# dkogan/libdogleg

Hardware: AMD Instinct MI355X
Metric: trust-region steps/sec (fp64) at fixed (Nmeas,Nstate,nnz) (higher is better)
Workload: dtype f64

## Files before the change

### libdogleg_amd/csrc/sparse_factor.hip

```cpp
#include "sparse_internal.h"
#include "panel_factor.h"
#include "factor_tail.h"

namespace {
#ifdef DLG_FL_PROFILE
constexpr int FL_PROF_WG = 4096;
__device__ long long g_fl_prof[32*FL_PROF_WG*8];
__device__ long long g_fl_add[FL_PROF_WG*4];
#define FL_ADD_STAMP(k) do { if(HANDOFF && threadIdx.x == 0 && blockIdx.x < FL_PROF_WG) g_fl_add[blockIdx.x*4 + (k)] = wall_clock64(); } while(0)
#define FL_STAMP(k) do { if(threadIdx.x == 0 && blockIdx.x < FL_PROF_WG) g_fl_prof[((prof_lvl & 31)*FL_PROF_WG + blockIdx.x)*8 + (k)] = wall_clock64(); } while(0)
#else
#define FL_STAMP(k)
#define FL_ADD_STAMP(k)
#endif

template <int NT, bool UT_LDS, bool HANDOFF = false>
__device__ __forceinline__ void mf_add_children(double* P, double* Wt, int ntri, int nch, int ch0,
                                                MfChild rc, const MfChild* __restrict__ mf_rec,
                                                const double* uscr, const uint16_t* __restrict__ mf_dst, int tid,
                                                int* pr_flag = nullptr, int pr_epoch = 0, DlgHandoff ho = DlgHandoff{nullptr, 0, 0}, int z0 = 0)
{
  constexpr int MF_SLOTS = (NT >= 512) ? 20 : 16;
  const int lane = tid & 63;
  for(int e = z0 + tid; e < ntri; e += NT) Wt[e] = 0.0;
// ... 513 lines not shown
  const double* Ld = Lx + sn_lx[d] + wd;
  double* U = uscr + u_off[d];
  const int T = (mb + 15) >> 4, MB16 = T*16;
  const int LDB = ((mb + 31)/32)*32 + 16, K4 = (wd + 3) & ~3;
  const int tid = threadIdx.x, lane = tid & 63;
  const int w = __builtin_amdgcn_readfirstlane(tid >> 6);
  const int jn = lane & 15, kq = lane >> 4;
  const int ntiles = T*(T + 1)/2;
  int aoff[TPW], boff[TPW];
#pragma unroll
  for(int q = 0; q < TPW; q++)
  {
    int rem = w + q*NW, tj = 0;
    if(rem < ntiles) { while(rem >= T - tj) { rem -= T - tj; tj++; } }
    else { rem = 0; tj = 0; }
    aoff[q] = 16*(tj + rem); boff[q] = 16*tj;
  }
  const int nmine = (ntiles - w + NW - 1)/NW;
  dlg_v4d c4[TPW];
#pragma unroll
  for(int q = 0; q < TPW; q++) c4[q] = (dlg_v4d){0.0, 0.0, 0.0, 0.0};
  for(int k0 = 0; k0 < K4; k0 += KC)
  {
    const int kc = min(KC, K4 - k0);
    if(k0 > 0) __syncthreads();
    batched_copy<NT, 8>(kc*MB16, tid,
                        [&](int e) { const int k = k0 + e / MB16, i = e % MB16; return (k < wd && i < mb) ? Ld[i + (size_t)k*nrows] : 0.0; },
                        [&](int e, double v) { const int k = e / MB16, i = e - k*MB16; Bs[k*LDB + i] = v; });
    __syncthreads();
    const double* base = Bs + kq*LDB + jn;
#pragma unroll 2
    for(int kk = 0; kk < kc; kk += 4)
    {
#pragma unroll
      for(int q = 0; q < TPW; q++)
        if(q < nmine)
          c4[q] = __builtin_amdgcn_mfma_f64_16x16x4f64(base[kk*LDB + aoff[q]], base[kk*LDB + boff[q]], c4[q], 0, 0, 0);
    }
  }
#pragma unroll
  for(int q = 0; q < TPW; q++)
    if(q < nmine)
    {
      const int j = boff[q] + jn;
#pragma unroll
      for(int r = 0; r < 4; r++)
      {
        const int i = aoff[q] + kq + 4*r;
        if(i < mb && j <= i) U[tri_col(j, mb) + i] = c4[q][r];
      }
    }
}
constexpr int GATHER_FLIGHT = 4;
template <int NT>
__global__ void __launch_bounds__(NT) k_update_gather(int unit0, const GatherUnit* __restrict__ units,
                                                       const SymSub* __restrict__ usub,
                                                       const int64_t* __restrict__ usub_u,
                                                       const int* __restrict__ relpos,
                                                       double* __restrict__ Lx,
                                                       double* __restrict__ upart,
                                                       const double* __restrict__ uscr, int nw,
                                                       int* __restrict__ info,
                                                       const int* __restrict__ fin_gate = nullptr, int fin_epoch = 0, int* fin_status = nullptr)
{
  extern __shared__ __attribute__((aligned(16))) double lds[];
  __shared__ int s_skip;
  int fin_seen = fin_epoch;
  if(fin_gate && threadIdx.x == 0) fin_seen = __hip_atomic_load(fin_gate, __ATOMIC_RELAXED, __HIP_MEMORY_SCOPE_AGENT);
  if(threadIdx.x == 0)
  {
    s_skip = *info != 0x7fffffff;
  }
  const GatherUnit U0 = units[unit0 + blockIdx.x];
  const int nc = U0.nc, nrows_t = U0.nrows_t, s0 = U0.s0, s1 = U0.s1;
  double* Lt = Lx + U0.lt;
  const int64_t part = U0.part;
  const int tid = threadIdx.x, lane = tid & 63;
  const int w = __builtin_amdgcn_readfirstlane(tid >> 6);
  const int slab = nrows_t*nc;
  for(int e = tid; e < slab*nw; e += NT) lds[e] = 0.0;
  __syncthreads();
  if(s_skip) return;
  if(w < nw)
  {
    double* acc = lds + (size_t)w*slab;
    const int nmine = (s1 - s0 - w + nw - 1)/nw;
    for(int k0 = 0; k0 < nmine; k0 += 64)
    {
      const int stl = s0 + w + (k0 + min(lane, nmine - k0 - 1))*nw;
      const SymSub R = usub[stl];
      const int64_t ru = usub_u[stl];
      const int r_rel = R.rel, r_mb = R.nrows_d - R.wd, r_m = R.m;
      const int r_ulo = (int)(uint32_t)ru, r_uhi = (int)(ru >> 32);
      const int nb = min(64, nmine - k0);
      for(int k = 0; k < nb; k += GATHER_FLIGHT)
      {
        int relv[GATHER_FLIGHT], mbv[GATHER_FLIGHT], mv[GATHER_FLIGHT], mmax = 0;
        const double* Uv[GATHER_FLIGHT];
#pragma unroll
        for(int g = 0; g < GATHER_FLIGHT; g++)
        {
          const int kg = min(k + g, nb - 1);
          relv[g] = __builtin_amdgcn_readlane(r_rel, kg);
          mbv[g] = __builtin_amdgcn_readlane(r_mb, kg);
          mv[g] = (k + g < nb) ? __builtin_amdgcn_readlane(r_m, kg) : 0;
          Uv[g] = uscr + (int64_t)(((uint64_t)(uint32_t)__builtin_amdgcn_readlane(r_uhi, kg) << 32) | (uint32_t)__builtin_amdgcn_readlane(r_ulo, kg));
          mmax = max(mmax, mv[g]);
        }
        int mv2[GATHER_FLIGHT];
#pragma unroll
        for(int g = 0; g < GATHER_FLIGHT; g++) mv2[g] = max(mv[g], 1);
        for(int i0 = 0; i0 < mmax; i0 += 64)
        {
          const int i = i0 + lane;
          const int cmax = (i < nc - 1) ? i : nc - 1;
          int ig[GATHER_FLIGHT], rg[GATHER_FLIGHT];
          double v[GATHER_FLIGHT][8];
#pragma unroll
          for(int g = 0; g < GATHER_FLIGHT; g++) { ig[g] = min(i, max(mv[g], 1) - 1); rg[g] = relpos[relv[g] + ig[g]]; }
#pragma unroll
          for(int g = 0; g < GATHER_FLIGHT; g++)
#pragma unroll
            for(int c = 0; c < 8; c++)
              if(c < nc) { const int cc = min(min(c, cmax), ig[g]); v[g][c] = Uv[g][ig[g] + cc*(mv2[g] - 1) - cc*(cc - 1)/2]; }
#pragma unroll
          for(int g = 0; g < GATHER_FLIGHT; g++)
#pragma unroll
            for(int c = 0; c < 8; c++)
              if(c < nc) { if(i < mv[g] && c <= cmax) acc[rg[g] + c*nrows_t] += v[g][c]; }
        }
      }
    }
  }
  if(fin_gate && tid == 0)
    for(int spins = 0; fin_seen != fin_epoch; spins++)
    {
      if(spins > (1 << 21)) { atomicOr(fin_status, DLG_HANDOFF_FACTOR); break; }
      __builtin_amdgcn_s_sleep(8);
      fin_seen = __hip_atomic_load(fin_gate, __ATOMIC_ACQUIRE, __HIP_MEMORY_SCOPE_AGENT);
    }
  __syncthreads();
  for(int e0 = tid; e0 < slab; e0 += 8*NT)
  {
    double old[8], tot[8];
#pragma unroll
    for(int u = 0; u < 8; u++) old[u] = (part < 0 && e0 + u*NT < slab) ? Lt[e0 + u*NT] : 0.0;
#pragma unroll
    for(int u = 0; u < 8; u++)
    {
      tot[u] = 0.0;
      if(e0 + u*NT < slab) for(int k = 0; k < nw; k++) tot[u] += lds[(size_t)k*slab + e0 + u*NT];
    }
#pragma unroll
    for(int u = 0; u < 8; u++)
      if(e0 + u*NT < slab) { if(part < 0) Lt[e0 + u*NT] = old[u] - tot[u]; else upart[part + e0 + u*NT] = tot[u]; }
  }
}

constexpr int UPD_TILES = 6;
__global__ void __launch_bounds__(TPB) k_update_mfma(int unit0, const int* __restrict__ uw_item,
                                                     const int* __restrict__ uw_s0,
                                                     const int* __restrict__ uw_s1,
                                                     const int64_t* __restrict__ uw_part,
                                                     const int* __restrict__ ui_t,
                                                     const int* __restrict__ ui_col,
                                                     const int* __restrict__ ui_nc,
                                                     const SymSub* __restrict__ usub,
                                                     const int* __restrict__ relpos,
                                                     const int* __restrict__ sn_rowptr,
                                                     const int64_t* __restrict__ sn_lx,
                                                     double* __restrict__ Lx,
                                                     double* __restrict__ upart, int nw, const int* __restrict__ info)
{
  extern __shared__ __attribute__((aligned(16))) double lds[];
  if(*info != 0x7fffffff) return;

  const int unit = unit0 + blockIdx.x;
  const int item = uw_item[unit];
  const int t = ui_t[item], col = ui_col[item], nc = ui_nc[item];
  const int nrows_t = sn_rowptr[t+1] - sn_rowptr[t];
  double* Lt = Lx + sn_lx[t] + (int64_t)col*nrows_t;
  const int s0 = uw_s0[unit], s1 = uw_s1[unit];
  const int64_t part = uw_part[unit];
  const int tid = threadIdx.x, lane = tid & 63;
  const int w = __builtin_amdgcn_readfirstlane(tid >> 6);
  const int slab = nrows_t*nc;
  for(int e = tid; e < slab*nw; e += TPB) lds[e] = 0.0;
  __syncthreads();
  if(w < nw)
  {
    double* acc = lds + (size_t)w*slab;
    const int jn = lane & 15, kq = lane >> 4;
    const int jc = min(jn, nc - 1);
    int piece = 0;
    for(int st = s0; st < s1; st++)
    {
      const SymSub U = usub[st];
      const double* Ld = Lx + U.src;
      const int* rel = relpos + U.rel;
      const int ld = U.nrows_d, wd = U.wd, m = U.m;
      for(int mt0 = 0; mt0 < m; mt0 += 16*UPD_TILES, piece++)
      {
        if(piece % nw != w) continue;
        const int ntile = min(UPD_TILES, (m - mt0 + 15) >> 4);
        const int relv0 = rel[min(mt0 + lane, m - 1)], relv1 = rel[min(mt0 + 64 + lane, m - 1)];
        dlg_v4d c4[UPD_TILES];
#pragma unroll
        for(int q = 0; q < UPD_TILES; q++) c4[q] = (dlg_v4d){0.0, 0.0, 0.0, 0.0};
        int ia[UPD_TILES];
// ... 100 lines not shown
            const double ai = Ld[i + (size_t)q*ld];
#pragma unroll
            for(int c = 0; c < 8; c++) if(c <= cmax) sacc[c] += ai*Ld[c + (size_t)q*ld];
          }
          const int r = rel[i];
#pragma unroll
          for(int c = 0; c < 8; c++) if(c <= cmax) acc[r + c*nrows_t] += sacc[c];
        }
      }
    }
    __syncthreads();
    for(int e = tid; e < slab; e += TPB)
    {
      double tot = 0.0;
      for(int k = 0; k < nw; k++) tot += lds[(size_t)k*slab + e];
      if(part < 0) Lt[e] -= tot; else upart[part + e] = tot;
    }
  }
  else
  {
    double* dst = (part < 0) ? Lt : upart + part;
    const double sgn = (part < 0) ? -1.0 : 1.0;
    if(part >= 0) { for(int e = tid; e < slab; e += TPB) dst[e] = 0.0; __syncthreads(); }
    for(int st = s0; st < s1; st++)
    {
      const SymSub U = usub[st];
      const double* Ld = Lx + U.src;
      const int* rel = relpos + U.rel;
      const int ld = U.nrows_d;
      for(int i = tid; i < U.m; i += TPB)
      {
        const int cmax = (i < nc - 1) ? i : nc - 1;
        const int r = rel[i];
        for(int c = 0; c <= cmax; c++)
        {
          double sacc = 0.0;
          for(int q = 0; q < U.wd; q++) sacc += Ld[i + (size_t)q*ld]*Ld[c + (size_t)q*ld];
          dst[r + c*nrows_t] += sgn*sacc;
        }
      }
      __syncthreads();
    }
  }
}
__global__ void __launch_bounds__(TPB) k_update_fin(int f0, const int* __restrict__ uf_item,
                                                    const int* __restrict__ uf_n,
                                                    const int64_t* __restrict__ uf_off,
                                                    const int* __restrict__ ui_t,
                                                    const int* __restrict__ ui_col,
                                                    const int* __restrict__ ui_nc,
                                                    const int* __restrict__ sn_rowptr,
                                                    const int64_t* __restrict__ sn_lx,
                                                    double* __restrict__ Lx,
                                                    const double* __restrict__ upart, const int* __restrict__ info)
{
  __shared__ double sh[TPB];
  if(*info != 0x7fffffff) return;

  const int f = f0 + blockIdx.x;
  const int item = uf_item[f], n = uf_n[f];
  const int t = ui_t[item], col = ui_col[item], nc = ui_nc[item];
  const int nrows_t = sn_rowptr[t+1] - sn_rowptr[t];
  double* Lt = Lx + sn_lx[t] + (int64_t)col*nrows_t;
  const int slab = nrows_t*nc;
  const double* src = upart + uf_off[f];
  const int E = (slab >= 32) ? 32 : 8;
  const int G = TPB/E;
  const int el = threadIdx.x % E, g = threadIdx.x / E;
  for(int ebase = blockIdx.y*E; ebase < slab; ebase += gridDim.y*E)
  {
    const int e = ebase + el;
    double t0 = 0.0, t1 = 0.0, t2 = 0.0, t3 = 0.0;
    if(e < slab)
    {
      const double* q = src + e;
      int k = g;
      for(; k + 3*G < n; k += 4*G)
      {
        t0 += q[(size_t)k*slab];         t1 += q[(size_t)(k + G)*slab];
        t2 += q[(size_t)(k + 2*G)*slab]; t3 += q[(size_t)(k + 3*G)*slab];
      }
      for(; k < n; k += G) t0 += q[(size_t)k*slab];
    }
    __syncthreads();
    sh[threadIdx.x] = (t0 + t1) + (t2 + t3);
    __syncthreads();
    if(g == 0 && e < slab)
    {
      double sacc = 0.0;
      for(int k = 0; k < G; k++) sacc += sh[k*E + el];
      Lt[e] -= sacc;
    }
  }
}

}

static int env_int_host(const char* n, int d) { const char* v = getenv(n); return v ? atoi(v) : d; }
int sparse_factor_setup(dlg_backend* b, bool plan_only)
{
  SparseSym* Y = b->sym;
  const SymHost& H = Y->H;
  Y->fac_b16 = true;
  Y->fac_lds.assign(H.nlevels, 0); Y->fac_nt.assign(H.nlevels, 512); Y->upd_coop.assign(H.nlevels, 0);
  Y->upd_lds.assign(H.nlevels, 0); Y->upd_nw.assign(H.nlevels, 0);
  Y->syrk_lds.assign(H.nlevels, 0); Y->syrk_nt.assign(H.nlevels, 256); Y->syrk_kc.assign(H.nlevels, 4);
  Y->syrk_fused.assign(H.nlevels, 0); Y->fin_ny.assign(H.nlevels, 1); Y->fac_stage.assign(H.nlevels, 0);
  Y->fac_leaf.assign(H.nlevels, 0);
  for(int l = 0; l < H.nlevels && !getenv("DOGLEG_AMD_NO_LEAF_KERNEL"); l++)
  {
    bool all = H.fw_lvl_ptr[l+1] > H.fw_lvl_ptr[l] && l < H.mf_level0;
    long maxr = 0;
// ... 53 lines not shown
    if(H.upd_syrk[l])
    {
      long ldbmax = 0, k4max = 0, tmax = 0;
      for(int i = H.lvl_ptr[l]; i < H.lvl_ptr[l+1]; i++)
      {
        const int d = H.lvl_sn[i];
        const long wd = H.sn_c0[d+1] - H.sn_c0[d], mb = H.sn_rowptr[d+1] - H.sn_rowptr[d] - wd;
        ldbmax = std::max(ldbmax, ((mb + 31)/32)*32 + 16); k4max = std::max(k4max, (wd + 3)/4*4);
        tmax = std::max(tmax, (mb + 15)/16);
      }
      long kc = (65536/(ldbmax*8)) & ~3L;
      if(kc > k4max) kc = k4max;
      Y->syrk_kc[l] = (int)kc;
      Y->syrk_lds[l] = (int)(kc*ldbmax*8);
      Y->syrk_nt[l] = (tmax*(tmax + 1)/2 <= 32) ? 256 : 1024;
      bool unsliced = true;
      for(int i = H.lvl_ptr[l]; i < H.lvl_ptr[l+1]; i++) if(H.sn_top[H.lvl_sn[i]] >= 0) unsliced = false;
      Y->syrk_fused[l] = (unsliced && nw > 0 && !getenv("DOGLEG_AMD_NO_SYRK_FUSE")) ? 1 : 0;
    }
    if(l >= H.mf_level0 || Y->syrk_fused[l])
    {
      long with_children = Y->fac_lds[l], leaves = Y->fac_lds[l];
      for(int i = H.lvl_ptr[l]; i < H.lvl_ptr[l+1]; i++)
      {
        const int s = H.lvl_sn[i];
        const long wv = H.sn_c0[s+1] - H.sn_c0[s], nr = H.sn_rowptr[s+1] - H.sn_rowptr[s], mb = nr - wv;
        const bool cmp = H.sn_bd_ptr[s+1] > H.sn_bd_ptr[s] && H.sn_top[s] < 0;
        const long pan = cmp ? ((mb + 1) & ~1L)*wv + (Y->fac_leaf[l] ? 4 : 8)*wv : ((nr + 1) & ~1L)*wv;
        const int jsp = cmp ? (int)mb : sym_w_split(wv, nr);
        const long need = (pan + (jsp >= 0 ? sym_w_linear(mb, jsp) : mb*(mb + 1)/2) + 1)*8;
        const long need0 = (pan + 1)*8;
        const long want = (need <= FAC_LDS_BUDGET && jsp >= 0) ? need : need0;
        const bool has_children = l >= H.mf_level0 && H.mf_cptr[s+1] > H.mf_cptr[s];
        if(has_children) with_children = std::max(with_children, want); else leaves = std::max(leaves, want);
      }
      const long base = std::max((long)Y->fac_lds[l], with_children);
      const long per_cu0 = 163840/(base + 3584), per_cu1 = 163840/(std::max(base, leaves) + 3584);
      Y->fac_stage[l] = (per_cu1 == per_cu0) ? 1 : 0;
      Y->fac_lds[l] = (int)(Y->fac_stage[l] ? std::max(base, leaves) : base);
    }
    if(getenv("DOGLEG_AMD_SYM_DEBUG"))
      fprintf(stderr, "factor level %d: %d supernodes, dynamic LDS %d bytes, update matrices staged %d, leaf instantiation %d, gather: %d waves, %d bytes\n",
              l, H.lvl_ptr[l+1] - H.lvl_ptr[l], Y->fac_lds[l], (int)Y->fac_stage[l], (int)Y->fac_leaf[l], Y->upd_nw[l], Y->upd_lds[l]);
  }
  if(!Y->uw_flat && !H.uw_item.empty() && !plan_only)
  {
    std::vector<GatherUnit> fl(H.uw_item.size());
    for(size_t u = 0; u < fl.size(); u++)
    {
      const int item = H.uw_item[u], t = H.ui_t[item];
      const int nr = H.sn_rowptr[t+1] - H.sn_rowptr[t];
      fl[u].lt = H.sn_lx[t] + (int64_t)H.ui_col[item]*nr; fl[u].part = H.uw_part[u];
      fl[u].s0 = H.uw_s0[u]; fl[u].s1 = H.uw_s1[u]; fl[u].nrows_t = nr; fl[u].nc = H.ui_nc[item];
    }
    DLG_CHECK(upload(Y->uw_flat, fl)); Y->allocs.push_back(Y->uw_flat);
  }
  Y->pr_level0 = H.nlevels; Y->pr2_level0 = H.nlevels; Y->pr2_level1 = -1;
  const bool dbg = getenv("DOGLEG_AMD_TIMING") != nullptr;
  bool acc_any = false;
  auto build_region = [&](int lo_min, int hi, int& r_level0, int& r_lds, int& r_stage, int& r_nwg,
                          std::vector<FwItem>& items, std::vector<MfChild>& rec, std::vector<uint16_t>& dst) -> int
  {
    r_level0 = H.nlevels; r_nwg = 0;
    if(getenv("DOGLEG_AMD_NO_PERSIST") || H.nlevels < 2 || hi < lo_min) return DLG_OK;
    const int ncu = b->ncu;
    const int cap = env_int_host("DOGLEG_AMD_PERSIST_MAX", 5*ncu);
    int total = 0, l0 = hi + 1, lds = 0, stage = 1;
    const int nt = Y->fac_nt[hi];
    for(int l = hi; l >= std::max(1, lo_min); l--)
    {
      const int n = H.fw_lvl_ptr[l+1] - H.fw_lvl_ptr[l];
      if(l < H.mf_level0) break;
      if(n == 0 || total + n > cap || Y->fac_nt[l] != nt || Y->fac_lds[l] <= 0) break;
      if(H.uw_lvl_ptr[l+1] > H.uw_lvl_ptr[l] || H.uf_lvl_ptr[l+1] > H.uf_lvl_ptr[l]) break;
      bool ok = true;
      for(int i = H.fw_lvl_ptr[l]; i < H.fw_lvl_ptr[l+1] && ok; i++)
      {
        const FwItem& it = H.fw_item[i];
        if(it.top >= 0 || it.r0 != 0 || it.nbd > 0) ok = false;
      }
      if(!ok) break;
      stage = stage && Y->fac_stage[l]; total += n; l0 = l; lds = std::max(lds, Y->fac_lds[l]);
    }
    if(hi + 1 - l0 < 2) return DLG_OK;
    r_level0 = l0; r_lds = lds; r_stage = stage;
    {
      const int rmax = std::max(1, std::min(8, env_int_host("DOGLEG_AMD_FRONT_REPLICAS", 8)));
      const int fill = ncu/2, fill0 = ncu/2;
      const bool slice_ok = !getenv("DOGLEG_AMD_NO_FRONT_SLICES");
      std::vector<int> first(H.fw_item.size(), -1), count(H.fw_item.size(), 0);
      rec = H.mf_rec; dst = H.mf_dst;
      auto lin = [](long j, long mb) { return j*mb - j*(j - 1)/2; };
      long lds_need = lds;
      std::vector<double> est(H.fw_item.size(), 0.0);
      std::vector<int> item_of_sn(H.nsn, -1);
      for(int l = r_level0; l <= hi; l++)
        for(int i = H.fw_lvl_ptr[l]; i < H.fw_lvl_ptr[l+1]; i++) item_of_sn[H.fw_sn[i]] = i;
      for(int l = r_level0; l <= hi; l++)
      {
        const int n = H.fw_lvl_ptr[l+1] - H.fw_lvl_ptr[l];
        std::vector<int> order(n);
        for(int k = 0; k < n; k++) order[k] = H.fw_lvl_ptr[l] + k;
        for(int i : order)
        {
          const FwItem& fi = H.fw_item[i];
          double e0 = 0.0;
// ... 171 lines not shown
      std::vector<FwItem> items2; std::vector<MfChild> rec2; std::vector<uint16_t> dst2;
      DLG_CHECK(build_region(1, H.cut_level, Y->pr2_level0, Y->pr2_lds, Y->pr2_stage, Y->pr2_nwg, items2, rec2, dst2));
      if(Y->pr2_level0 <= H.cut_level)
      {
        Y->pr2_level1 = H.cut_level;
        if(!Y->pr2_item) { DLG_CHECK(upload(Y->pr2_item, items2)); Y->allocs.push_back(Y->pr2_item); }
        if(!Y->pr2_rec)  { DLG_CHECK(upload(Y->pr2_rec, rec2));   Y->allocs.push_back(Y->pr2_rec); }
        if(!Y->pr2_dst)  { DLG_CHECK(upload(Y->pr2_dst, dst2));   Y->allocs.push_back(Y->pr2_dst); }
      }
      else Y->pr2_level0 = H.nlevels;
    }
    if(acc_any && !Y->pr_acc && !plan_only)
    {
      DLG_HIP(hipMalloc(&Y->pr_acc, sizeof(double)*(size_t)std::max<int64_t>(1, H.uscr_size)));
      Y->allocs.push_back(Y->pr_acc);
    }
  }
  if(plan_only) return DLG_OK;
  if(Y->pr_level0 < H.nlevels && !Y->fac_flag)
  {
    DLG_HIP(hipMalloc(&Y->fac_flag, sizeof(int)*((size_t)Y->pr_nwg + 1)));
    Y->allocs.push_back(Y->fac_flag);
    DLG_HIP(hipMemsetAsync(Y->fac_flag, 0, sizeof(int)*((size_t)Y->pr_nwg + 1), b->stream));
    Y->fac_epoch = 0;
  }
  if(Y->pr2_level0 < H.nlevels && !Y->fac2_flag)
  {
    DLG_HIP(hipMalloc(&Y->fac2_flag, sizeof(int)*((size_t)Y->pr2_nwg + 1)));
    Y->allocs.push_back(Y->fac2_flag);
    DLG_HIP(hipMemsetAsync(Y->fac2_flag, 0, sizeof(int)*((size_t)Y->pr2_nwg + 1), b->stream));
    Y->fac2_epoch = 0;
  }
  DLG_HIP(hipFuncSetAttribute(reinterpret_cast<const void*>(&k_factor_level<128>),
                              hipFuncAttributeMaxDynamicSharedMemorySize, FAC_LDS_BUDGET));
  DLG_HIP(hipFuncSetAttribute(reinterpret_cast<const void*>(&k_factor_level<256>),
                              hipFuncAttributeMaxDynamicSharedMemorySize, FAC_LDS_BUDGET));
  DLG_HIP(hipFuncSetAttribute(reinterpret_cast<const void*>(&k_factor_level<256, true>),
                              hipFuncAttributeMaxDynamicSharedMemorySize, FAC_LDS_BUDGET));
  DLG_HIP(hipFuncSetAttribute(reinterpret_cast<const void*>(&k_factor_level<512>),
                              hipFuncAttributeMaxDynamicSharedMemorySize, FAC_LDS_BUDGET));
  DLG_HIP(hipFuncSetAttribute(reinterpret_cast<const void*>(&k_update_level),
                              hipFuncAttributeMaxDynamicSharedMemorySize, LDS_BUDGET));
  DLG_HIP(hipFuncSetAttribute(reinterpret_cast<const void*>(&k_update_syrk<256>),
                              hipFuncAttributeMaxDynamicSharedMemorySize, LDS_BUDGET));
  DLG_HIP(hipFuncSetAttribute(reinterpret_cast<const void*>(&k_update_syrk<1024>),
                              hipFuncAttributeMaxDynamicSharedMemorySize, LDS_BUDGET));
  DLG_HIP(hipFuncSetAttribute(reinterpret_cast<const void*>(&k_update_gather<TPB>),
                              hipFuncAttributeMaxDynamicSharedMemorySize, LDS_BUDGET));
  DLG_HIP(hipFuncSetAttribute(reinterpret_cast<const void*>(&k_update_mfma),
                              hipFuncAttributeMaxDynamicSharedMemorySize, LDS_BUDGET));
  return DLG_OK;
}

#ifdef DLG_FL_PROFILE
extern "C" void dlg_fl_profile_dump(int nlevels)
{
  std::vector<long long> h(32*FL_PROF_WG*8);
  hipDeviceSynchronize();
  hipMemcpyFromSymbol(h.data(), HIP_SYMBOL(g_fl_prof), sizeof(long long)*h.size());
  for(int l = 0; l < nlevels && l < 32; l++)
  {
    int nwg = 0, last = -1; long long t0 = 0, tend = 0; double mean[5] = {0, 0, 0, 0, 0};
    for(int g = 0; g < FL_PROF_WG; g++)
    {
      const long long* q = &h[(l*FL_PROF_WG + g)*8];
      if(q[5] == 0) continue;
      nwg++;
      if(t0 == 0 || q[0] < t0) t0 = q[0];
      if(q[5] > tend) { tend = q[5]; last = g; }
      for(int k = 0; k < 5; k++) mean[k] += (double)(q[k+1] - q[k]);
    }
    if(nwg == 0) continue;
    for(int g = FL_PROF_WG - 1, shown = 0; g >= 0 && shown < (getenv("DLG_FL_DUMP_ALL") ? FL_PROF_WG : 20); g--)
    {
      const long long* q = &h[(l*FL_PROF_WG + g)*8];
      if(q[5] == 0 || q[7] == 0) continue;
      shown++;
      {
        std::vector<long long> ha(FL_PROF_WG*4);
        static bool got = false; static std::vector<long long> hadd;
        if(!got) { hadd.resize(FL_PROF_WG*4); hipMemcpyFromSymbol(hadd.data(), HIP_SYMBOL(g_fl_add), sizeof(long long)*hadd.size()); got = true; }
        if(hadd[g*4 + 0]) fprintf(stderr, "   add %3d: child0 seen %6lld child0 added %6lld last child seen %6lld dbg %lld\n", g, hadd[g*4] - t0, hadd[g*4 + 1] - t0, hadd[g*4 + 2] - t0, hadd[g*4 + 3]);
      }
      fprintf(stderr, "   wg %3d (w %3lld rows %4lld nch %lld u_lds %lld lvl %lld rep %lld): start %6lld flag up %6lld panel in %6lld added %6lld factored %6lld tail %6lld flag+stored %6lld\n",
              g, q[6] & 4095, (q[6] >> 12) & 4095, (q[6] >> 24) & 4095, (q[6] >> 36) & 1, (q[6] >> 56) & 63, (q[6] >> 52) & 15, q[0] - t0, q[7] - t0, q[1] - t0, q[2] - t0, q[3] - t0, q[4] - t0, q[5] - t0);
    }
    const long long* q = &h[(l*FL_PROF_WG + last)*8];
    fprintf(stderr, "level %2d: %3d wg, span %7lld | last wg %3d (w %3lld rows %4lld slice %4lld nch %2lld u_lds %lld has_u %lld): start +%6lld load %6lld add %6lld factor %6lld tail %6lld store %6lld | mean: load %6.0f add %6.0f factor %6.0f tail %6.0f store %6.0f\n",
            l, nwg, tend - t0, last, q[6] & 4095, (q[6] >> 12) & 4095, (q[6] >> 40) & 4095, (q[6] >> 24) & 4095, (q[6] >> 36) & 1, (q[6] >> 37) & 1,
            q[0] - t0, q[1] - q[0], q[2] - q[1], q[3] - q[2], q[4] - q[3], q[5] - q[4],
            mean[0]/nwg, mean[1]/nwg, mean[2]/nwg, mean[3]/nwg, mean[4]/nwg);
  }
  std::vector<long long> z(h.size(), 0);
  hipMemcpyToSymbol(HIP_SYMBOL(g_fl_prof), z.data(), sizeof(long long)*z.size());
}
#endif
int sparse_factor_levels(dlg_backend* b, int part)
{
  SparseSym* Y = b->sym;
  const SymHost& H = Y->H;
  hipStream_t st = b->stream;
  const bool split = Y->pr_level0 > 0 && H.nlevels >= 2 && H.part_nranks <= 1 && H.fw_lvl_ptr[1] > H.fw_lvl_ptr[0];
  if(part == 2 && !split) return DLG_OK;
  if(part != 2)
  {
  if(H.part_nranks > 1 && H.cut_level < 0) DLG_CHECK(sparse_partition_reduce(b));
// ... 40 lines not shown
      const DlgHandoff ho = dlg_handoff(b, 1 << 21);
      DlgRegionTurn turn(b);
      if(Y->fac_nt[l] == 128)
        hipLaunchKernelGGL(HIP_KERNEL_NAME(k_factor_level<128>), dim3(np), dim3(128), Y->pr_lds, st,
                           Y->pr_item, Y->pr_rec, Y->sn_bd_col, Y->pr_dst, Y->Lx, Y->top_scr, Y->d_info, Y->uscr, fmode, fl, ep, ho, pacc);
      else if(Y->fac_nt[l] == 256)
        hipLaunchKernelGGL(HIP_KERNEL_NAME(k_factor_level<256>), dim3(np), dim3(256), Y->pr_lds, st,
                           Y->pr_item, Y->pr_rec, Y->sn_bd_col, Y->pr_dst, Y->Lx, Y->top_scr, Y->d_info, Y->uscr, fmode, fl, ep, ho, pacc);
      else
        hipLaunchKernelGGL(HIP_KERNEL_NAME(k_factor_level<512>), dim3(np), dim3(512), Y->pr_lds, st,
                           Y->pr_item, Y->pr_rec, Y->sn_bd_col, Y->pr_dst, Y->Lx, Y->top_scr, Y->d_info, Y->uscr, fmode, fl, ep, ho, pacc);
      break;
    }
    if(n > 0 && !launched_before)
    {
      const int o = H.fw_lvl_ptr[l];
      const int sweep_bits = (Y->fac_b16 ? 16 : 0);
      const int fmode = ((l >= H.mf_level0) ? 2 : Y->syrk_fused[l]) + 4*Y->fac_stage[l] + sweep_bits + 256*(l & 31);
      if(Y->fac_nt[l] == 128)
        hipLaunchKernelGGL(HIP_KERNEL_NAME(k_factor_level<128>), dim3(n), dim3(128), Y->fac_lds[l], st,
                           Y->fw_item + o, Y->mf_rec, Y->sn_bd_col, Y->mf_dst, Y->Lx, Y->top_scr, Y->d_info, Y->uscr, fmode, (int*)nullptr, 0, DlgHandoff{nullptr, 0, 0}, (int64_t)0);
      else if(Y->fac_nt[l] == 256 && Y->fac_leaf[l])
        hipLaunchKernelGGL(HIP_KERNEL_NAME(k_factor_level<256, true>), dim3(n), dim3(256), Y->fac_lds[l], st,
                           Y->fw_item + o, Y->mf_rec, Y->sn_bd_col, Y->mf_dst, Y->Lx, Y->top_scr, Y->d_info, Y->uscr, fmode, (int*)nullptr, 0, DlgHandoff{nullptr, 0, 0}, (int64_t)0);
      else if(Y->fac_nt[l] == 256)
        hipLaunchKernelGGL(HIP_KERNEL_NAME(k_factor_level<256>), dim3(n), dim3(256), Y->fac_lds[l], st,
                           Y->fw_item + o, Y->mf_rec, Y->sn_bd_col, Y->mf_dst, Y->Lx, Y->top_scr, Y->d_info, Y->uscr, fmode, (int*)nullptr, 0, DlgHandoff{nullptr, 0, 0}, (int64_t)0);
      else
        hipLaunchKernelGGL(HIP_KERNEL_NAME(k_factor_level<512>), dim3(n), dim3(512), Y->fac_lds[l], st,
                           Y->fw_item + o, Y->mf_rec, Y->sn_bd_col, Y->mf_dst, Y->Lx, Y->top_scr, Y->d_info, Y->uscr, fmode, (int*)nullptr, 0, DlgHandoff{nullptr, 0, 0}, (int64_t)0);
    }
    if(part == 1 && split && l == 0) { Y->fac_pending = true; DLG_LAUNCH_CHECK(); return DLG_OK; }
    const int nu = H.uw_lvl_ptr[l+1] - H.uw_lvl_ptr[l];
    const bool gather_next = nu > 0 && H.upd_syrk[l] && Y->upd_nw[l] > 0;
    const int fin_ep = (l == 0 && gather_next) ? Y->fin_side_owed : 0;
    if(fin_ep) Y->fin_side_owed = 0;
    if(l == 0) DLG_CHECK(sparse_fin_side_gate(b));
    if(gather_next)
    {
      const int ns = H.xl_ptr[l+1] - H.xl_ptr[l];
      if(Y->syrk_fused[l] || ns == 0) {  }
      else if(Y->syrk_nt[l] == 256)
        hipLaunchKernelGGL(HIP_KERNEL_NAME(k_update_syrk<256>), dim3(ns), dim3(256), Y->syrk_lds[l], st,
                           Y->xl_sn + H.xl_ptr[l], Y->sn_c0, Y->sn_rowptr, Y->sn_lx, Y->u_off, Y->Lx, Y->uscr,
                           Y->syrk_kc[l]);
      else
        hipLaunchKernelGGL(HIP_KERNEL_NAME(k_update_syrk<1024>), dim3(ns), dim3(1024), Y->syrk_lds[l], st,
                           Y->xl_sn + H.xl_ptr[l], Y->sn_c0, Y->sn_rowptr, Y->sn_lx, Y->u_off, Y->Lx, Y->uscr,
                           Y->syrk_kc[l]);
      hipLaunchKernelGGL(HIP_KERNEL_NAME(k_update_gather<TPB>), dim3(nu), dim3(TPB), Y->upd_lds[l], st, H.uw_lvl_ptr[l],
                         Y->uw_flat, Y->usub, Y->usub_u, Y->relpos, Y->Lx, Y->upart, Y->uscr,
                         Y->upd_nw[l], Y->d_info,
                         fin_ep ? (const int*)(Y->fin_flag + 1) : (const int*)nullptr, fin_ep,
                         reinterpret_cast<int*>(b->d_scal + (dlg_backend::NSCAL - 2)));
    }
    else if(nu > 0 && Y->upd_coop[l] == 2)
      hipLaunchKernelGGL(k_update_mfma, dim3(nu), dim3(TPB), Y->upd_lds[l], st, H.uw_lvl_ptr[l],
                         Y->uw_item, Y->uw_s0, Y->uw_s1, Y->uw_part, Y->ui_t, Y->ui_col, Y->ui_nc,
                         Y->usub, Y->relpos, Y->sn_rowptr, Y->sn_lx, Y->Lx, Y->upart, Y->upd_nw[l], (const int*)Y->d_info);
    else if(nu > 0 && Y->upd_coop[l])
      hipLaunchKernelGGL(k_update_coop, dim3(nu), dim3(TPB), 0, st, H.uw_lvl_ptr[l],
                         Y->uw_item, Y->uw_s0, Y->uw_s1, Y->uw_part, Y->ui_t, Y->ui_col, Y->ui_nc,
                         Y->usub, Y->relpos, Y->sn_rowptr, Y->sn_lx, Y->Lx, Y->upart, (const int*)Y->d_info);
    else if(nu > 0)
      hipLaunchKernelGGL(k_update_level, dim3(nu), dim3(TPB), Y->upd_lds[l], st, H.uw_lvl_ptr[l],
                         Y->uw_item, Y->uw_s0, Y->uw_s1, Y->uw_part, Y->ui_t, Y->ui_col, Y->ui_nc,
                         Y->usub, Y->relpos, Y->sn_rowptr, Y->sn_lx, Y->Lx, Y->upart, Y->upd_nw[l], (const int*)Y->d_info);
    const int nfz = H.uf_lvl_ptr[l+1] - H.uf_lvl_ptr[l];
    if(nfz > 0)
      hipLaunchKernelGGL(k_update_fin, dim3(nfz, Y->fin_ny[l]), dim3(TPB), 0, st, H.uf_lvl_ptr[l], Y->uf_item, Y->uf_n,
                         Y->uf_off, Y->ui_t, Y->ui_col, Y->ui_nc, Y->sn_rowptr, Y->sn_lx, Y->Lx,
                         Y->upart, (const int*)Y->d_info);
    if(H.part_nranks > 1 && l == H.cut_level) { DLG_LAUNCH_CHECK(); DLG_CHECK(sparse_partition_reduce(b)); }
  }
  if(!H.ms_sn.empty())
    hipLaunchKernelGGL(k_copy_top, dim3((unsigned)H.ms_sn.size()), dim3(TPB), 0, st, Y->ms_sn, Y->sn_c0,
                       Y->sn_rowptr, Y->sn_lx, Y->sn_top, Y->Lx, Y->top_scr, (const int*)Y->d_info);
  DLG_LAUNCH_CHECK();
  return DLG_OK;
}

extern "C" int dlg_sparse_region_probe(int N, int M, const int* colptr, const int* rowidx, int ncu, long* stats, int nstats)
{
  dlg_backend b;
  b.type = DLG_SPARSE; b.N = N; b.M = M; b.nnz = colptr[M]; b.ncu = ncu; b.row0 = 0; b.row1 = M; b.mloc = M;
  SparseSym Y;
  b.sym = &Y;
  char err[512];
  if(sym_analyze(Y.H, N, M, colptr, rowidx, 0, M, err, sizeof(err))) { b.sym = nullptr; dlg_set_error("symbolic analysis: %s", err); return DLG_ERR_ARG; }
  const int rc = sparse_factor_setup(&b, true);
  b.sym = nullptr;
  if(rc != DLG_OK) return rc;
  const SymHost& H = Y.H;
  long nsliced = 0, nhbm = 0;
  auto fail = [&](const char* what, size_t g) { dlg_set_error("one-launch region: %s (workgroup %zu)", what, g); return DLG_ERR_STATE; };
  std::vector<long> covered;
  for(size_t g = 0; g < Y.pr_item_h.size(); g++)
  {
    const FwItem& it = Y.pr_item_h[g];
    const long mb = it.nrows - it.w, ldp = (it.nrows + 1) & ~1L, pan = ldp*it.w, ntri = mb*(mb + 1)/2;
    const long T = (mb + 15) >> 4;
    if(it.rep == 0) covered.assign((size_t)std::max<long>(T, 1), 0);
    for(long t = std::min<long>(it.tj0, T); t < std::min<long>(it.tj1, T); t++) covered[(size_t)t]++;
    long lds_end;
    if(it.sliced)
    {
      nsliced++;
      const long jA = std::min<long>(16L*it.tj0, mb), jB = it.tj1 >= T ? mb : std::min<long>(16L*it.tj1, mb);
      if(it.eA != jA*mb - jA*(jA - 1)/2 || it.eB != jB*mb - jB*(jB - 1)/2) return fail("slice bounds do not match its tile columns", g);
      lds_end = pan + (it.eA & 1) + (it.eB - it.eA) + 1;
    }
    else
    {
      if(it.jsp < 0 && mb > 0 && it.u_off >= 0)
      {
        if(it.rep == 0) nhbm++;
        if(it.rsv2 > 1)
        {
          const long jA = std::min<long>(16L*it.tj0, mb), jB = it.tj1 >= T ? mb : std::min<long>(16L*it.tj1, mb);
          if(it.eA != jA*mb - jA*(jA - 1)/2 || it.eB != jB*mb - jB*(jB - 1)/2) return fail("an HBM replica's stretch does not match its tile columns", g);
        }
        else if(it.tj0 != 0 || it.tj1 < T) return fail("a single workgroup that does not form the whole update matrix", g);
      }
      const bool staged = it.jsp >= 0 && mb > 0 && it.u_off >= 0 && (it.nch > 0 || Y.pr_stage);
      lds_end = pan + (staged ? sym_w_linear(mb, it.jsp) : 0) + 1;
// ... 32 lines not shown
```

### libdogleg_amd/csrc/sparse_internal.h

```cpp
#pragma once
#include "dlg_internal.h"
#include "sparse_symbolic.h"

namespace {
constexpr int JFL_SEG = 16;
constexpr int NV_CHUNK = 2048;

constexpr int TPB = 256;
constexpr int LDS_BUDGET = 147456;
constexpr int FAC_LDS_BUDGET = SYM_FAC_LDS_BUDGET;

__device__ __forceinline__ double wave_sum(double v)
{
#pragma unroll
  for(int o = 32; o > 0; o >>= 1) v += __shfl_down(v, o, 64);
  return v;
}

template <int NT, int U, class LoadF, class StoreF>
__device__ __forceinline__ void batched_copy(int total, int tid, LoadF ld, StoreF st)
{
  for(int base = 0; base < total; base += U*NT)
  {
    double v[U];
#pragma unroll
    for(int u = 0; u < U; u++) { const int idx = base + u*NT + tid; v[u] = (idx < total) ? ld(idx) : 0.0; }
#pragma unroll
    for(int u = 0; u < U; u++) { const int idx = base + u*NT + tid; if(idx < total) st(idx, v[u]); }
  }
}

template <class T> int upload(T*& dev, const std::vector<T>& h)
{
  dev = nullptr;
  const size_t bytes = sizeof(T)*(h.size() ? h.size() : 1);
  DLG_HIP(hipMalloc(&dev, bytes));
  if(!h.empty()) DLG_HIP(hipMemcpy(dev, h.data(), sizeof(T)*h.size(), hipMemcpyHostToDevice));
  return DLG_OK;
}

}

struct GatherUnit { int64_t lt, part; int s0, s1, nrows_t, nc; };
struct SolveItem { int c0, w, nrows, rowoff; int64_t lx; int bd0, nbd; int pflag, rsv; };

struct SparseSym
{
  SymHost H;
  uint64_t pat_key = 0;
  int *sn_c0 = nullptr, *sn_rowptr = nullptr, *sn_rows = nullptr, *sn_scr = nullptr, *lvl_sn = nullptr;
  int64_t *sn_lx = nullptr, *diagpos = nullptr;
  int *ui_t = nullptr, *ui_col = nullptr, *ui_nc = nullptr, *ui_ptr = nullptr;
  SymSub* usub = nullptr; int* relpos = nullptr;
  int *uw_item = nullptr, *uw_s0 = nullptr, *uw_s1 = nullptr, *uf_item = nullptr, *uf_n = nullptr;
  int64_t *uw_part = nullptr, *uf_off = nullptr;
  GatherUnit* uw_flat = nullptr;
  double* upart = nullptr; double* uscr = nullptr; int64_t *u_off = nullptr, *usub_u = nullptr;
  SolveItem* slv_item = nullptr; FwItem* fw_item = nullptr; MfChild* mf_rec = nullptr; uint16_t* mf_dst = nullptr;
  SymOutBlock* oblk = nullptr; SymContrib* contrib = nullptr;
  SymTask *jtx_task = nullptr;
  int *jtx_fin_ptr = nullptr, *jtx_fin_blk = nullptr;
  int *jtx_fin_short = nullptr, *jtx_fin_long = nullptr; int n_fin_short = 0, n_fin_long = 0;
  AsmRho* asm_rho = nullptr; AsmPair* asm_pair = nullptr; AsmSlot* asm_slot = nullptr;
  AsmBatch* asm_batch = nullptr; AsmTask* asm_ctask = nullptr; AsmFin* asm_cfin = nullptr;
  bool asm_pent_ok = false;
  uint32_t* asm_pent = nullptr;
  AsmShape* asm_shape = nullptr; AsmKG* asm_kg = nullptr; AsmMTask* asm_mtask = nullptr; int* asm_tdest = nullptr;
  int *jf_ptr = nullptr, *jf_ent = nullptr, *jf_var0 = nullptr, *jf_w = nullptr, *jf_short = nullptr, *jf_long = nullptr;
  double* jf_lpart = nullptr; int* jf_lcnt = nullptr;
  const double* fin_pending_rhs = nullptr; const double* spec_aug_rhs = nullptr; bool info_clean = false;
  double* fin_pending_Lx = nullptr;
  bool spare_dirty = false, spare_zeroed = false; hipStream_t spare_stream = nullptr;
  double* jtp = nullptr;
  AsmFin2* asm_fin2 = nullptr; int64_t* asm_fin2_list = nullptr; AsmRun* asm_run = nullptr; int* asm_pdest = nullptr;
  int *rl_ptr = nullptr, *rl_pos = nullptr, *perm = nullptr, *col_sn = nullptr;
  int *fw_sn = nullptr, *fw_r0 = nullptr, *fw_r1 = nullptr, *ms_sn = nullptr; int64_t* sn_top = nullptr;
  int *sn_bd_ptr = nullptr, *sn_bd_col = nullptr;
  double* top_scr = nullptr;
  const double* aug_rhs = nullptr;
  int *Jp = nullptr, *Ji = nullptr;
  int *gat_rows = nullptr, *gat_src = nullptr;
  int *nv_chunk = nullptr; int n_nv_chunks = 0;
  double *Lx = nullptr, *scr = nullptr, *ywork = nullptr, *asm_part = nullptr, *jtx_part = nullptr;
  int *d_info = nullptr, *h_info = nullptr;
  bool info_armed = false;
  bool zero_fail_seen = false; int64_t* leaf_diag = nullptr; int* leaf_diag_col = nullptr; int n_leaf_diag = 0;
  double* intact_Lx = nullptr; const double* intact_J = nullptr; int intact_slot = -1; double intact_lambda = 0.0;
  const double* fac_J = nullptr; int fac_slot = -1;
  bool fac_pending = false;
  size_t nnz_loc = 0;
  uint32_t* ar_idx = nullptr; double* ar_buf = nullptr; size_t ar_n = 0;
  std::vector<int> fac_lds;
  std::vector<int> upd_lds, upd_nw, slv_lds, bwd_lds, fac_nt, upd_coop, syrk_lds, syrk_nt, syrk_kc, bwd_nt, syrk_fused, fin_ny, fac_stage, bwd_top, bwd_bd, bwd_pmx, fac_leaf;
  int64_t* red_off = nullptr; int* red_len = nullptr; int* red_kind = nullptr; int64_t* red_dst = nullptr;
  int n_red_seg = 0; size_t red_n = 0; double* red_buf = nullptr;
  double* colmask = nullptr; int* sn_owner = nullptr;
  int64_t* augpos = nullptr;
  int *xl_sn = nullptr;
  double* held_Lx = nullptr; const double* held_aug = nullptr; double held_lambda = 0.0;
  double cur_lambda = 0.0;
  double *ms_scr = nullptr, *ms_y = nullptr; int ms_lds_f = 0, ms_lds_b = 0;
  typedef ReachPlan LevPlan;
  LevPlan lev[2];
  int* lev_iperm = nullptr; std::vector<int> lev_jp, lev_ji; int lev_lds = 0;
  double* Lx_spec = nullptr; hipEvent_t ev_spec = nullptr, ev_spec_fork = nullptr;
  bool spec_inflight = false, spec_valid = false; int spec_slot = -1; const double* spec_J = nullptr;
  int64_t touch_off = 0, touch_n = 0;
  int bw_level0 = 1 << 30, bw_lds = 0, bw_n = 0;
  SolveItem* slv_item_pr = nullptr; int* bwd_flag = nullptr; int bwd_epoch = 0; double* bwd_xh = nullptr;
// ... 28 lines not shown
```

Before: 1850.

## Fold multi-chunk update reduction into gather kernel via per-item arrival counters

Gather workgroups that write partial update chunks for an item now count their arrival on a per-item atomic counter. Once all of an item's chunks are written, each participating workgroup sums a strided share of the partials and subtracts it from L, and k_update_fin skips folded items or is not launched at all. This targets the extra k_update_fin launch and the kernel boundary between gather and reduction. In exchange it adds spin-waits that require every unit of an item to be co-resident (hence the occupancy check), atomic stores and loads on the partials, and layout reordering of gather units.

```diff
diff --git a/libdogleg_amd/csrc/sparse_factor.hip b/libdogleg_amd/csrc/sparse_factor.hip
--- a/libdogleg_amd/csrc/sparse_factor.hip
+++ b/libdogleg_amd/csrc/sparse_factor.hip
@@ -589,6 +589,9 @@
     }
 }
 constexpr int GATHER_FLIGHT = 4;
+#ifdef DLG_GATHER_STATS
+__device__ unsigned long long g_gather_stats[8];
+#endif
 template <int NT>
 __global__ void __launch_bounds__(NT) k_update_gather(int unit0, const GatherUnit* __restrict__ units,
                                                        const SymSub* __restrict__ usub,
@@ -598,10 +601,12 @@
                                                        double* __restrict__ upart,
                                                        const double* __restrict__ uscr, int nw,
                                                        int* __restrict__ info,
-                                                       const int* __restrict__ fin_gate = nullptr, int fin_epoch = 0, int* fin_status = nullptr)
+                                                       const int* __restrict__ fin_gate = nullptr, int fin_epoch = 0, int* fin_status = nullptr,
+                                                       int* __restrict__ fin_cnt = nullptr)
 {
   extern __shared__ __attribute__((aligned(16))) double lds[];
-  __shared__ int s_skip;
+  __shared__ int s_skip, s_last;
+  typedef __attribute__((address_space(1))) double* gdp_t;
   int fin_seen = fin_epoch;
   if(fin_gate && threadIdx.x == 0) fin_seen = __hip_atomic_load(fin_gate, __ATOMIC_RELAXED, __HIP_MEMORY_SCOPE_AGENT);
   if(threadIdx.x == 0)
@@ -617,7 +622,13 @@
   const int slab = nrows_t*nc;
   for(int e = tid; e < slab*nw; e += NT) lds[e] = 0.0;
   __syncthreads();
-  if(s_skip) return;
+  if(s_skip)
+  {
+    const int fn = units[unit0 + blockIdx.x].fin_n, ff = units[unit0 + blockIdx.x].fin_f;
+    if(fn > 0 && tid == 0 && (atomicAdd(fin_cnt + ff, 0x10001) >> 16) == fn - 1)
+      __hip_atomic_store(fin_cnt + ff, 0, __ATOMIC_RELAXED, __HIP_MEMORY_SCOPE_AGENT);
+    return;
+  }
   if(w < nw)
   {
     double* acc = lds + (size_t)w*slab;
@@ -669,6 +680,10 @@
       }
     }
   }
+#ifdef DLG_GATHER_STATS
+  const bool gs_down = fin_gate && tid == 0 && fin_seen != fin_epoch;
+  const long long gs_t0 = gs_down ? (long long)wall_clock64() : 0;
+#endif
   if(fin_gate && tid == 0)
     for(int spins = 0; fin_seen != fin_epoch; spins++)
     {
@@ -676,7 +691,20 @@
       __builtin_amdgcn_s_sleep(8);
       fin_seen = __hip_atomic_load(fin_gate, __ATOMIC_ACQUIRE, __HIP_MEMORY_SCOPE_AGENT);
     }
+#ifdef DLG_GATHER_STATS
+  if(fin_gate && tid == 0)
+  {
+    atomicAdd(&g_gather_stats[0], 1ull);
+    if(blockIdx.x == 0) atomicAdd(&g_gather_stats[4], 1ull);
+    if(gs_down)
+    {
+      const unsigned long long dt = (unsigned long long)((long long)wall_clock64() - gs_t0);
+      atomicAdd(&g_gather_stats[1], 1ull); atomicAdd(&g_gather_stats[2], dt); atomicMax(&g_gather_stats[3], dt);
+    }
+  }
+#endif
   __syncthreads();
+  const int fin_n = units[unit0 + blockIdx.x].fin_n;
   for(int e0 = tid; e0 < slab; e0 += 8*NT)
   {
     double old[8], tot[8];
@@ -690,8 +718,68 @@
     }
 #pragma unroll
     for(int u = 0; u < 8; u++)
-      if(e0 + u*NT < slab) { if(part < 0) Lt[e0 + u*NT] = old[u] - tot[u]; else upart[part + e0 + u*NT] = tot[u]; }
-  }
+      if(e0 + u*NT < slab)
+      {
+        if(part < 0) Lt[e0 + u*NT] = old[u] - tot[u];
+        else if(fin_n > 0) __hip_atomic_store((gdp_t)(upart + part + e0 + u*NT), tot[u], __ATOMIC_RELAXED, __HIP_MEMORY_SCOPE_AGENT);
+        else upart[part + e0 + u*NT] = tot[u];
+      }
+  }
+  if(fin_n <= 0) return;
+  asm volatile("s_waitcnt vmcnt(0)" ::: "memory");
+  __syncthreads();
+  int* cnt = fin_cnt + units[unit0 + blockIdx.x].fin_f;
+  if(tid == 0)
+  {
+    atomicAdd(cnt, 1);
+    for(int spins = 0; (__hip_atomic_load(cnt, __ATOMIC_RELAXED, __HIP_MEMORY_SCOPE_AGENT) & 0xffff) < fin_n; spins++)
+    {
+      if(spins > (1 << 21)) { atomicOr(fin_status, DLG_HANDOFF_FACTOR); break; }
+      __builtin_amdgcn_s_sleep(8);
+    }
+    (void)__hip_atomic_load(cnt, __ATOMIC_ACQUIRE, __HIP_MEMORY_SCOPE_AGENT);
+    s_last = __hip_atomic_load(info, __ATOMIC_RELAXED, __HIP_MEMORY_SCOPE_AGENT) == 0x7fffffff;
+  }
+  __syncthreads();
+  if(s_last)
+  {
+    static_assert(NT == TPB, "the folded k_update_fin sums in k_update_fin's thread groups");
+    const int fin_k = units[unit0 + blockIdx.x].fin_k;
+    const double* src = upart + (part - (int64_t)fin_k*slab);
+    const int E = (slab >= 32) ? 32 : 8;
+    const int G = NT/E;
+    const int el = tid % E, g = tid / E;
+    for(int ebase = fin_k*E; ebase < slab; ebase += fin_n*E)
+    {
+      const int e = ebase + el;
+      double t0 = 0.0, t1 = 0.0, t2 = 0.0, t3 = 0.0;
+      if(e < slab)
+      {
+        const double* q = src + e;
+        int k = g;
+        for(; k + 3*G < fin_n; k += 4*G)
+        {
+          t0 += __hip_atomic_load((gdp_t)(q + (size_t)k*slab), __ATOMIC_RELAXED, __HIP_MEMORY_SCOPE_AGENT);
+          t1 += __hip_atomic_load((gdp_t)(q + (size_t)(k + G)*slab), __ATOMIC_RELAXED, __HIP_MEMORY_SCOPE_AGENT);
+          t2 += __hip_atomic_load((gdp_t)(q + (size_t)(k + 2*G)*slab), __ATOMIC_RELAXED, __HIP_MEMORY_SCOPE_AGENT);
+          t3 += __hip_atomic_load((gdp_t)(q + (size_t)(k + 3*G)*slab), __ATOMIC_RELAXED, __HIP_MEMORY_SCOPE_AGENT);
+        }
+        for(; k < fin_n; k += G) t0 += __hip_atomic_load((gdp_t)(q + (size_t)k*slab), __ATOMIC_RELAXED, __HIP_MEMORY_SCOPE_AGENT);
+      }
+      __syncthreads();
+      lds[tid] = (t0 + t1) + (t2 + t3);
+      __syncthreads();
+      if(g == 0 && e < slab)
+      {
+        double sacc = 0.0;
+        for(int k = 0; k < G; k++) sacc += lds[k*E + el];
+        Lt[e] -= sacc;
+      }
+    }
+  }
+  __syncthreads();
+  if(tid == 0 && (atomicAdd(cnt, 0x10000) >> 16) == fin_n - 1)
+    __hip_atomic_store(cnt, 0, __ATOMIC_RELAXED, __HIP_MEMORY_SCOPE_AGENT);
 }
 
 constexpr int UPD_TILES = 6;
@@ -898,12 +986,14 @@
                                                     const int* __restrict__ sn_rowptr,
                                                     const int64_t* __restrict__ sn_lx,
                                                     double* __restrict__ Lx,
-                                                    const double* __restrict__ upart, const int* __restrict__ info)
+                                                    const double* __restrict__ upart, const int* __restrict__ info,
+                                                    const int* __restrict__ uf_fold = nullptr)
 {
   __shared__ double sh[TPB];
   if(*info != 0x7fffffff) return;
 
   const int f = f0 + blockIdx.x;
+  if(uf_fold && uf_fold[f]) return;
   const int item = uf_item[f], n = uf_n[f];
   const int t = ui_t[item], col = ui_col[item], nc = ui_nc[item];
   const int nrows_t = sn_rowptr[t+1] - sn_rowptr[t];
@@ -1063,6 +1153,54 @@
       const int nr = H.sn_rowptr[t+1] - H.sn_rowptr[t];
       fl[u].lt = H.sn_lx[t] + (int64_t)H.ui_col[item]*nr; fl[u].part = H.uw_part[u];
       fl[u].s0 = H.uw_s0[u]; fl[u].s1 = H.uw_s1[u]; fl[u].nrows_t = nr; fl[u].nc = H.ui_nc[item];
+      fl[u].fin_n = 0; fl[u].fin_k = 0; fl[u].fin_f = 0; fl[u].rsv = 0;
+    }
+    Y->fin_left.assign(H.nlevels, 0);
+    for(int l = 0; l < H.nlevels; l++) Y->fin_left[l] = H.uf_lvl_ptr[l+1] - H.uf_lvl_ptr[l];
+    std::vector<int> fold(H.uf_item.size(), 0);
+    bool any_fold = false;
+    if(!getenv("DOGLEG_AMD_NO_GATHER_FIN") && H.part_nranks <= 1 && !b->sharded())
+    {
+      const bool any_size = getenv("DOGLEG_AMD_DEBUG_GATHER_FIN_ANY_SIZE") != nullptr;
+      std::vector<int> f_of_item(H.ui_t.size(), -1);
+      for(size_t f = 0; f < H.uf_item.size(); f++) f_of_item[H.uf_item[f]] = (int)f;
+      for(int l = 0; l < H.nlevels; l++)
+      {
+        const int u0 = H.uw_lvl_ptr[l], u1 = H.uw_lvl_ptr[l+1], nu = u1 - u0;
+        if(!(nu > 0 && H.upd_syrk[l] && Y->upd_nw[l] > 0) || Y->fin_left[l] == 0) continue;
+        if(Y->upd_lds[l] < (int)(TPB*sizeof(double))) continue;
+        int per_cu = 0;
+        (void)hipFuncSetAttribute(reinterpret_cast<const void*>(&k_update_gather<TPB>), hipFuncAttributeMaxDynamicSharedMemorySize, LDS_BUDGET);
+        if(hipOccupancyMaxActiveBlocksPerMultiprocessor(&per_cu, k_update_gather<TPB>, TPB, (size_t)Y->upd_lds[l]) != hipSuccess) { (void)hipGetLastError(); continue; }
+        if(per_cu <= 0 || ((long)nu < 2L*per_cu*b->ncu && !any_size)) continue;
+        for(int f = H.uf_lvl_ptr[l]; f < H.uf_lvl_ptr[l+1]; f++)
+        {
+          if(H.uf_n[f] <= std::min(32767L, (long)per_cu*b->ncu/8)) { fold[f] = 1; Y->fin_left[l]--; any_fold = true; }
+        }
+        std::vector<GatherUnit> front, back;
+        for(int u = u0; u < u1; u++)
+        {
+          const int f = H.uw_part[u] >= 0 ? f_of_item[H.uw_item[u]] : -1;
+          if(f >= 0 && fold[f])
+          {
+            const int64_t slab = (int64_t)fl[u].nrows_t*fl[u].nc;
+            fl[u].fin_n = H.uf_n[f]; fl[u].fin_k = (int)((H.uw_part[u] - H.uf_off[f])/slab); fl[u].fin_f = f;
+            front.push_back(fl[u]);
+          }
+          else back.push_back(fl[u]);
+        }
+        if(getenv("DOGLEG_AMD_SYM_DEBUG"))
+          fprintf(stderr, "gather fin: level %d, %d units (%d resident), %d of %d multi-chunk items summed by their own %d units\n",
+                  l, nu, per_cu*b->ncu, (H.uf_lvl_ptr[l+1] - H.uf_lvl_ptr[l]) - Y->fin_left[l], H.uf_lvl_ptr[l+1] - H.uf_lvl_ptr[l], (int)front.size());
+        std::copy(front.begin(), front.end(), fl.begin() + u0);
+        std::copy(back.begin(), back.end(), fl.begin() + u0 + (long)front.size());
+      }
+    }
+    if(any_fold)
+    {
+      DLG_CHECK(upload(Y->uf_fold, fold)); Y->allocs.push_back(Y->uf_fold);
+      DLG_HIP(hipMalloc(&Y->fin_cnt, sizeof(int)*fold.size())); Y->allocs.push_back(Y->fin_cnt);
+      DLG_HIP(hipMemset(Y->fin_cnt, 0, sizeof(int)*fold.size()));
     }
     DLG_CHECK(upload(Y->uw_flat, fl)); Y->allocs.push_back(Y->uw_flat);
   }
@@ -1340,6 +1478,17 @@
   return DLG_OK;
 }
 
+#ifdef DLG_GATHER_STATS
+extern "C" void dlg_gather_stats_dump(void)
+{
+  unsigned long long h[8] = {0}, z[8] = {0};
+  (void)hipDeviceSynchronize();
+  (void)hipMemcpyFromSymbol(h, HIP_SYMBOL(g_gather_stats), sizeof(h));
+  (void)hipMemcpyToSymbol(HIP_SYMBOL(g_gather_stats), z, sizeof(z));
+  fprintf(stderr, "gather flag-B wait: %llu launches, %llu workgroups looked, %llu found the word down, their wait: mean %.2f us, max %.2f us, per launch %.2f workgroups waiting\n",
+          h[4], h[0], h[1], h[1] ? 0.01*(double)h[2]/(double)h[1] : 0.0, 0.01*(double)h[3], h[4] ? (double)h[1]/(double)h[4] : 0.0);
+}
+#endif
 #ifdef DLG_FL_PROFILE
 extern "C" void dlg_fl_profile_dump(int nlevels)
 {
@@ -1486,7 +1635,7 @@
                          Y->uw_flat, Y->usub, Y->usub_u, Y->relpos, Y->Lx, Y->upart, Y->uscr,
                          Y->upd_nw[l], Y->d_info,
                          fin_ep ? (const int*)(Y->fin_flag + 1) : (const int*)nullptr, fin_ep,
-                         reinterpret_cast<int*>(b->d_scal + (dlg_backend::NSCAL - 2)));
+                         reinterpret_cast<int*>(b->d_scal + (dlg_backend::NSCAL - 2)), Y->fin_cnt);
     }
     else if(nu > 0 && Y->upd_coop[l] == 2)
       hipLaunchKernelGGL(k_update_mfma, dim3(nu), dim3(TPB), Y->upd_lds[l], st, H.uw_lvl_ptr[l],
@@ -1501,10 +1650,10 @@
                          Y->uw_item, Y->uw_s0, Y->uw_s1, Y->uw_part, Y->ui_t, Y->ui_col, Y->ui_nc,
                          Y->usub, Y->relpos, Y->sn_rowptr, Y->sn_lx, Y->Lx, Y->upart, Y->upd_nw[l], (const int*)Y->d_info);
     const int nfz = H.uf_lvl_ptr[l+1] - H.uf_lvl_ptr[l];
-    if(nfz > 0)
+    if(nfz > 0 && (Y->fin_left.empty() || Y->fin_left[l] > 0))
       hipLaunchKernelGGL(k_update_fin, dim3(nfz, Y->fin_ny[l]), dim3(TPB), 0, st, H.uf_lvl_ptr[l], Y->uf_item, Y->uf_n,
                          Y->uf_off, Y->ui_t, Y->ui_col, Y->ui_nc, Y->sn_rowptr, Y->sn_lx, Y->Lx,
-                         Y->upart, (const int*)Y->d_info);
+                         Y->upart, (const int*)Y->d_info, (const int*)Y->uf_fold);
     if(H.part_nranks > 1 && l == H.cut_level) { DLG_LAUNCH_CHECK(); DLG_CHECK(sparse_partition_reduce(b)); }
   }
   if(!H.ms_sn.empty())
diff --git a/libdogleg_amd/csrc/sparse_internal.h b/libdogleg_amd/csrc/sparse_internal.h
--- a/libdogleg_amd/csrc/sparse_internal.h
+++ b/libdogleg_amd/csrc/sparse_internal.h
@@ -41,7 +41,7 @@
 
 }
 
-struct GatherUnit { int64_t lt, part; int s0, s1, nrows_t, nc; };
+struct GatherUnit { int64_t lt, part; int s0, s1, nrows_t, nc; int fin_n, fin_k, fin_f, rsv; };
 struct SolveItem { int c0, w, nrows, rowoff; int64_t lx; int bd0, nbd; int pflag, rsv; };
 
 struct SparseSym
@@ -55,6 +55,7 @@
   int *uw_item = nullptr, *uw_s0 = nullptr, *uw_s1 = nullptr, *uf_item = nullptr, *uf_n = nullptr;
   int64_t *uw_part = nullptr, *uf_off = nullptr;
   GatherUnit* uw_flat = nullptr;
+  int *uf_fold = nullptr, *fin_cnt = nullptr; std::vector<int> fin_left;
   double* upart = nullptr; double* uscr = nullptr; int64_t *u_off = nullptr, *usub_u = nullptr;
   SolveItem* slv_item = nullptr; FwItem* fw_item = nullptr; MfChild* mf_rec = nullptr; uint16_t* mf_dst = nullptr;
   SymOutBlock* oblk = nullptr; SymContrib* contrib = nullptr;
```

Result: no change. 1858 (median of 2 runs) (+0.4%).
